# facebookresearch/DLRM-FlexFlow

Hardware: AMD Instinct MI355X
Metric: dlrm_training_samples_per_sec (higher is better)
Workload: dtype f32; 1 GPU; criteo-terabyte-shape: 26 tables (rows 39884406-39043-17289-7420-20263-3-7120-1543-63-38532951-2953546-403346-10-2208-11938-155-4-976-14-39979771-25641295-39664984-585935-12972-108-36), emb_dim 128, bag 1, bot 13-512-256-128, top 3456-1024-1024-512-256-1, cat interaction, SGD lr 0.01, MSE loss; global_batch=32768, per_gpu_batch=32768, parallelism=single GPU, hipGraph-replayed step, step_graph=True

## Files before the change

### dlrm_flexflow_amd/csrc/embedding.hip

```cpp
#include "emb_reduce.h"
#include "lr_state.h"

#include <type_traits>

namespace {

using namespace ffh_emb;

struct EmbArgs {
  ffh_emb_table t[FFH_MAX_TABLES];
  unsigned short* out16[FFH_MAX_TABLES];
  char* out3[FFH_MAX_TABLES];
  int   out3c[FFH_MAX_TABLES];
  int64_t batch;
  int     ntables;
  int     L;
  int     D;
  int     aggr;
  int64_t nt_rows;
};

template <int VEC, class WT> struct RowVec { typedef typename std::conditional<VEC == 4, float4, float>::type type; };
template <> struct RowVec<4, uint16_t> { typedef uint2 type; };
template <> struct RowVec<1, uint16_t> { typedef unsigned short type; };
template <int VEC, class WT>
__device__ __forceinline__ float row_elem(const typename RowVec<VEC, WT>::type& v, int k) {
  if constexpr (std::is_same<WT, float>::value) return reinterpret_cast<const float*>(&v)[k];
  else return ffh_bf16_to_f32(reinterpret_cast<const unsigned short*>(&v)[k]);
}

template <int VEC, int UNROLL, class WT = float>
__global__ __launch_bounds__(256) void emb_fwd_kernel(const EmbArgs a) {
  ffh_kernel_prio();
  using vec_t = typename RowVec<VEC, WT>::type;
  constexpr int NQ = VEC / 4;
  const ffh_emb_table tb = a.t[blockIdx.y];
  const WT* const wt = reinterpret_cast<const WT*>(tb.weight);
  unsigned short* const o16 = a.out16[blockIdx.y];
  char* const o3 = a.out3[blockIdx.y];
  const int o3c = a.out3c[blockIdx.y];
  const int D = a.D, L = a.L;
  const int nvec = D / VEC;
  const int lpr = nvec < 64 ? nvec : 64;
  const int rpw = 64 / lpr;
  const int lane = threadIdx.x & 63;
  const int wave = threadIdx.x >> 6;
  const int rsub = lane / lpr;
  const int c0 = lane - rsub * lpr;
  const bool active = rsub < rpw;
  const int64_t rows_per_block = (int64_t)(blockDim.x >> 6) * rpw * UNROLL;
  const float inv = 1.0f / (float)L;
  const bool avg = a.aggr == FFH_AGGR_MODE_AVG;

// ... 195 lines not shown
  if (vec == 4) hipLaunchKernelGGL((emb_fwd_kernel<4, U, WT>), grid, dim3(256), 0, as_stream(s), a);
  else hipLaunchKernelGGL((emb_fwd_kernel<1, U, WT>), grid, dim3(256), 0, as_stream(s), a);
  FFH_LAUNCH_CHECK(c, "emb_fwd_kernel");
  return FFH_OK;
}

extern "C" {

int ffh_embedding_fwd_multi(ffh_ctx* c, const ffh_emb_table* tables, int nt, int L, int D, int64_t batch, int aggr, ffh_stream s) {
  return emb_fwd_launch<float>(c, tables, nt, L, D, batch, aggr, s);
}

int ffh_embedding_fwd(ffh_ctx* c, const int64_t* idx, float* out, const float* weight, int L, int D, int64_t batch,
                      int64_t num_entries, int64_t out_ld, int aggr, ffh_stream s) {
  ffh_emb_table t{idx, const_cast<float*>(weight), out, num_entries, out_ld};
  return ffh_embedding_fwd_multi(c, &t, 1, L, D, batch, aggr, s);
}

int ffh_embedding_bwd_dense(ffh_ctx* c, const int64_t* idx, const float* g, float* wg, int L, int D, int64_t batch,
                            int64_t num_entries, int64_t gld, int aggr, ffh_stream s) {
  ffh_emb_table t{idx, wg, const_cast<float*>(g), num_entries, gld};
  int rc = validate_tables(c, &t, 1, L, D, batch, aggr, "embedding_bwd_dense");
  if (rc) return rc;
  if (batch == 0) return FFH_OK;
  hipLaunchKernelGGL(emb_bwd_dense_kernel, dim3(ffh_grid(batch * D, 256, 4096)), dim3(256), 0, as_stream(s),
                     idx, g, wg, L, D, batch, gld, aggr == FFH_AGGR_MODE_AVG ? 1 : 0);
  FFH_LAUNCH_CHECK(c, "emb_bwd_dense_kernel");
  return FFH_OK;
}

int ffh_embedding_localize_rows(ffh_ctx* c, const int64_t* idx, int64_t* local, int64_t n, int64_t row_begin, int64_t rows_local, ffh_stream s) {
  FFH_REQUIRE(c, n >= 0 && row_begin >= 0 && rows_local >= 0 && ((idx && local) || n == 0), "embedding_localize_rows: bad args");
  if (n == 0) return FFH_OK;
  hipLaunchKernelGGL(emb_localize_kernel, dim3(ffh_grid(n, 256)), dim3(256), 0, as_stream(s), idx, local, n, row_begin, rows_local);
  FFH_LAUNCH_CHECK(c, "embedding_localize_rows");
  return FFH_OK;
}

size_t ffh_embedding_bwd_workspace_bytes(int nt, int L, int D, int64_t batch) {
  if (nt <= 0 || L <= 0 || D <= 0 || batch <= 0) return 0;
  return bwd_layout(nt, L, D, batch).total;
}

struct Bf16Cfg { const ffh_bf16_rounding* r; Bf16Keys keys; };
typedef bool (*UpdateOfFn)(const UpdateLaunch&);
static constexpr UpdateOfFn kUpdateOf[2] = {emb_update_launch_f32, emb_update_launch_bf16};
static void set_bf16_keys(Bf16Keys& keys, Bf16AdamKeys& adam, const Bf16Cfg& b16, const ffh_emb_state* states, int nt, int kind) {
  if (kind != FFH_SPARSE_OPT_ADAM) { keys = b16.keys; return; }
  Bf16AdamKeys k;
  memset(&k, 0, sizeof k);
  for (int i = 0; i < nt; i++) { k.s1[i] = states[i].s1; k.table[i] = b16.keys.table[i]; k.col0[i] = b16.keys.col0[i]; }
  adam = k;
}
static int emb_bwd_phases(ffh_ctx* c, const ffh_emb_table* tables, int nt, int L, int D, int64_t batch,
                          int aggr, float lr, ffh_stream s, const bool do_sort, const bool do_apply,
                          const ffh_sparse_opt* opt = nullptr, const ffh_emb_state* states = nullptr, const Bf16Cfg* b16 = nullptr,
                          const ffh_lr_state* lr_block = nullptr) {
  int rc = validate_tables(c, tables, nt, L, D, batch, aggr, "embedding_bwd_sgd_fused");
  if (rc) return rc;
  OptP op{};
  op.lr = lr;
  if (b16 && do_apply) {
    const ffh_bf16_rounding* r = b16->r;
    if (!r) return ffh_fail(c, FFH_ERR_BAD_ARG, "embedding_bwd_bf16: null ffh_bf16_rounding");
    if (r->mode != FFH_BF16_ROUND_STOCHASTIC && r->mode != FFH_BF16_ROUND_NEAREST) return ffh_fail(c, FFH_ERR_BAD_ARG, "embedding_bwd_bf16: unknown rounding mode");
    if (r->mode == FFH_BF16_ROUND_STOCHASTIC && !r->counter) return ffh_fail(c, FFH_ERR_BAD_ARG, "embedding_bwd_bf16: stochastic rounding needs the update counter");
    op.sr_mode = r->mode; op.sr_seed = r->seed; op.sr_counter = r->counter;
  }
  op.nt_rows = (int64_t)FFH_LAB_INT("FFH_EMB_APPLY_NT_MB", 64) * (int64_t)(1 << 20) / ((int64_t)D * (b16 ? 2 : 4));
  int kind = FFH_SPARSE_OPT_SGD;
  RowRule rule = RowRule::Sgd;
  if (opt && do_apply) {
    kind = opt->kind;
    if (!row_rule_of(kind, &rule)) return ffh_fail(c, FFH_ERR_BAD_ARG, "embedding_bwd_opt: unknown ffh_sparse_opt.kind");
    if (b16 && (kind == FFH_SPARSE_OPT_SGD_MOMENTUM || kind == FFH_SPARSE_OPT_ADAM) && nt > FFH_BF16_MAX_STATEFUL_TABLES)
      return ffh_fail(c, FFH_ERR_BAD_ARG, "embedding_bwd_opt_multi_bf16: momentum / Adam take at most FFH_BF16_MAX_STATEFUL_TABLES (32) tables per call");
    op.lr = opt->lr; op.wd = opt->weight_decay; op.mom = opt->momentum; op.nesterov = opt->nesterov ? 1 : 0;
    op.b1 = opt->beta1; op.b2 = opt->beta2; op.eps = opt->epsilon; op.omb1 = 1.0f - opt->beta1; op.omb2 = 1.0f - opt->beta2;
    if (kind == FFH_SPARSE_OPT_SGD && (op.wd != 0.0f || op.mom != 0.0f)) return ffh_fail(c, FFH_ERR_BAD_ARG, "embedding_bwd_opt: FFH_SPARSE_OPT_SGD takes no weight decay / momentum (use FFH_SPARSE_OPT_SGD_MOMENTUM)");
    if (lr_block) { op.lr = 0.0f; opt_set_lr_src(op, ffh_lr_rate_ptr(lr_block, kind == FFH_SPARSE_OPT_ADAM)); }
    const bool need0 = kind == FFH_SPARSE_OPT_ADAM || kind == FFH_SPARSE_OPT_ADAGRAD || kind == FFH_SPARSE_OPT_ROWWISE_ADAGRAD || (kind == FFH_SPARSE_OPT_SGD_MOMENTUM && op.mom > 0.0f);
    for (int i = 0; i < nt && batch > 0; i++) {
      if (need0 && (!states || !states[i].s0)) return ffh_fail(c, FFH_ERR_BAD_ARG, "embedding_bwd_opt: optimizer state (s0) missing");
      if (kind == FFH_SPARSE_OPT_ADAM && !states[i].s1) return ffh_fail(c, FFH_ERR_BAD_ARG, "embedding_bwd_opt: optimizer state (s1) missing");
    }
  }
  if (nt == 0 || batch == 0) return FFH_OK;
  const int64_t N = batch * L;
  if (N >= (1LL << 31)) return ffh_fail(c, FFH_ERR_UNSUPPORTED, "embedding_bwd_sgd_fused: batch*in_dim >= 2^31");
  int64_t maxR = 1;
  for (int i = 0; i < nt; i++) maxR = tables[i].num_entries > maxR ? tables[i].num_entries : maxR;
  if (maxR > (1LL << 32)) return ffh_fail(c, FFH_ERR_UNSUPPORTED, "embedding_bwd_sgd_fused: num_entries > 2^32");
  bool v4 = can_vec4(tables, nt, D);
  for (int i = 0; i < nt && v4 && kind != FFH_SPARSE_OPT_SGD && kind != FFH_SPARSE_OPT_ROWWISE_ADAGRAD; i++)
    v4 = (!states[i].s0 || aligned16(states[i].s0)) && (kind == FFH_SPARSE_OPT_ADAGRAD || !states[i].s1 || aligned16(states[i].s1));
  const int nvec = v4 ? D / 4 : D;
  if ((nvec + 63) / 64 > kMaxChunks * 64) return ffh_fail(c, FFH_ERR_UNSUPPORTED, "embedding_bwd_sgd_fused: out_dim too large");
  if (kind == FFH_SPARSE_OPT_ROWWISE_ADAGRAD && (nvec + 63) / 64 > kMaxChunks)
    return ffh_fail(c, FFH_ERR_UNSUPPORTED, "embedding_bwd_opt: FFH_SPARSE_OPT_ROWWISE_ADAGRAD takes out_dim <= 1024 (16-byte form) / 256 (include/ff_hip_rowwise.h)");
  const BwdLayout lay = bwd_layout(nt, L, D, batch);
  if (!c->ws || c->ws_bytes < lay.total) return ffh_fail(c, FFH_ERR_WORKSPACE, "embedding_bwd_sgd_fused: workspace too small (ffh_embedding_bwd_workspace_bytes)");
  char* ws = (char*)c->ws;
  if (!aligned16(ws)) return ffh_fail(c, FFH_ERR_WORKSPACE, "embedding_bwd_sgd_fused: workspace must be 16-byte aligned");
  const int64_t sig[4] = {nt, L, D, batch};
  if (do_sort && do_apply) {
    if (c->emb_sorted_ws == c->ws) c->emb_sorted_ws = nullptr;
// ... 22 lines not shown
      while (tb < 32 && ((tables[i].num_entries - 1) >> tb) != 0) tb++;
      sm.npass[i] = (uint8_t)((tb + rb_s - 1) / rb_s);
    }
    sm.kp = (uint2*)(ws + lay.kp_a);
    sm.partial0 = (float*)(ws + lay.partial); sm.meta0 = (uint2*)(ws + lay.meta);
    sm.partial1 = (float*)(ws + lay.partial1); sm.meta1 = (uint2*)(ws + lay.meta1);
    sm.N = N; sm.nch0 = lay.nchunks; sm.nch1 = lay.nchunks1; sm.rb = rb_s; sm.L = L; sm.D = D;
    sm.avg = aggr == FFH_AGGR_MODE_AVG ? 1 : 0; sm.op = op;
    for (int i = 0; i < nt && kind != FFH_SPARSE_OPT_SGD; i++) { sm.s0[i] = states[i].s0; sm.s1[i] = states[i].s1; }
    if (b16) set_bf16_keys(sm.b16, sm.b16a, *b16, states, nt, kind);
    int tile = (int)((N + kSmallRedParts - 1) / kSmallRedParts);
    tile = (tile + FFH_EMB_CHUNK - 1) / FFH_EMB_CHUNK * FFH_EMB_CHUNK;
    sm.tile = tile < FFH_EMB_CHUNK ? FFH_EMB_CHUNK : tile;
    if (!kUpdateOf[b16 ? 1 : 0](UpdateLaunch{rule, v4, lr_block != nullptr, false, &sm, nullptr, dim3(nt), as_stream(s)}))
      return ffh_fail(c, FFH_ERR_UNSUPPORTED, "embedding_bwd: no small-batch kernel for this rule / weight type");
    FFH_LAUNCH_CHECK(c, "emb_sgd_small_kernel");
    return FFH_OK;
  }
  int bits = 1;
  while (bits < 32 && ((maxR - 1) >> bits) != 0) bits++;
  static const int msd_env = FFH_LAB_INT("FFH_EMB_MSD", 1);
  static const int msd_max_tables = FFH_LAB_INT("FFH_EMB_MSD_MAX_TABLES", FFH_MAX_TABLES);
  int mb = 4;
  while (mb < kMaxRadixBits && (N >> (mb + 1)) >= 32) mb++;
  const bool msd = msd_env != 0 && bits > kMaxRadixBits && N <= 65536 && (N >> mb) <= 128 && (msd_env == 2 || nt <= msd_max_tables) &&
                   (size_t)lay.nblk * kMaxRadix >= (size_t)lay.nchunks1;
  const int passes = msd ? 1 : (bits + kMaxRadixBits - 1) / kMaxRadixBits;
  const int rb = msd ? mb : (bits + passes - 1) / passes;
  if (msd) snprintf(c->emb_route, sizeof c->emb_route, "buckets:bits=%d", rb); else snprintf(c->emb_route, sizeof c->emb_route, "lsd:passes=%d", passes);

  SortArgs sa;
  memset(&sa, 0, sizeof sa);
  RedArgs ra;
  memset(&ra, 0, sizeof ra);
  for (int i = 0; i < nt; i++) {
    sa.idx[i] = tables[i].idx;
    int tb = 1;
    while (tb < 32 && ((tables[i].num_entries - 1) >> tb) != 0) tb++;
    const int np = msd ? 1 : (tb + rb - 1) / rb;
    sa.npass[i] = (uint8_t)np;
    ra.parity[i] = (uint8_t)(np & 1);
    sa.shift_t[i] = ra.shift_t[i] = (uint8_t)(msd && tb > rb ? tb - rb : 0);
  }
  sa.msd = msd ? 1 : 0;
  sa.bstart = (uint32_t*)(ws + lay.bstart);
  ra.bstart = sa.bstart; ra.nextkey = (uint32_t*)(ws + lay.hist); ra.radix = 1 << rb;
  sa.hist = (uint32_t*)(ws + lay.hist);
  sa.N = N; sa.nblk = lay.nblk; sa.bits = rb;
  sa.clear[0] = (uint32_t*)(ws + lay.meta1); sa.nclear[0] = 4 * lay.nchunks1;
  sa.clear[1] = (uint32_t*)(ws + lay.arrive); sa.nclear[1] = lay.nchunks1 + 1;
  uint2* kbuf[2] = {(uint2*)(ws + lay.kp_a), (uint2*)(ws + lay.kp_b)};
  dim3 sgrid((unsigned)lay.nblk, (unsigned)nt);
  const int E = sort_per_thread(nt, N);
  for (int p = 0; p < passes && do_sort; p++) {
    sa.shift = p * rb;
    sa.pass = p;
    sa.src = kbuf[p & 1];
    sa.dst = kbuf[(p + 1) & 1];
#define FFH_SORT_PASS(FIRSTV, EV)                                                                              \
    hipLaunchKernelGGL((radix_hist_kernel<FIRSTV, EV>), sgrid, dim3(kSortThreads), 0, as_stream(s), sa);      \
    hipLaunchKernelGGL((radix_scatter_kernel<FIRSTV, EV>), sgrid, dim3(kSortThreads), 0, as_stream(s), sa);
    if (p == 0) {
      switch (E) { case 1: FFH_SORT_PASS(true, 1) break; case 2: FFH_SORT_PASS(true, 2) break; case 4: FFH_SORT_PASS(true, 4) break; default: FFH_SORT_PASS(true, 8) break; }
    } else {
      switch (E) { case 1: FFH_SORT_PASS(false, 1) break; case 2: FFH_SORT_PASS(false, 2) break; case 4: FFH_SORT_PASS(false, 4) break; default: FFH_SORT_PASS(false, 8) break; }
    }
#undef FFH_SORT_PASS
  }
  FFH_LAUNCH_CHECK(c, "radix sort");
  if (!do_apply) return FFH_OK;

  for (int i = 0; i < nt; i++) ra.t[i] = tables[i];
  ra.kp[0] = kbuf[0]; ra.kp[1] = kbuf[1];
  ra.tile = reduce_tile(nt, N);
  {
    static const int msd_tile = FFH_LAB_INT("FFH_EMB_MSD_TILE", 0);
    if (msd && msd_tile >= 128 && msd_tile <= kRedTile && (msd_tile & (msd_tile - 1)) == 0) ra.tile = msd_tile;
  }
  ra.partial = (float*)(ws + lay.partial);
  ra.meta = (uint2*)(ws + lay.meta);
  ra.N = N; ra.nchunks = lay.nchunks; ra.L = L; ra.D = D;
  ra.avg = aggr == FFH_AGGR_MODE_AVG ? 1 : 0;
  ra.op = op;
  for (int i = 0; i < nt && kind != FFH_SPARSE_OPT_SGD; i++) { ra.s0[i] = states[i].s0; ra.s1[i] = states[i].s1; }
  if (b16) set_bf16_keys(ra.b16, ra.b16a, *b16, states, nt, kind);
  ra.partial1 = (float*)(ws + lay.partial1);
  ra.meta1 = (uint2*)(ws + lay.meta1); ra.nchunks1 = lay.nchunks1;
  ra.arrive = (uint32_t*)(ws + lay.arrive);
  dim3 rgrid((unsigned)((N + ra.tile - 1) / ra.tile), (unsigned)nt);
  if (!kUpdateOf[b16 ? 1 : 0](UpdateLaunch{rule, v4, lr_block != nullptr, msd, nullptr, &ra, rgrid, as_stream(s)}))
    return ffh_fail(c, FFH_ERR_UNSUPPORTED, "embedding_bwd: no reduce kernel for this rule / weight type");
  FFH_LAUNCH_CHECK(c, "emb_sgd_reduce/fold");
  return FFH_OK;
}

int ffh_embedding_bwd_sgd_fused_multi(ffh_ctx* c, const ffh_emb_table* tables, int nt, int L, int D, int64_t batch,
                                      int aggr, float lr, ffh_stream s) {
  return emb_bwd_phases(c, tables, nt, L, D, batch, aggr, lr, s, true, true);
}

int ffh_embedding_bwd_sort_multi(ffh_ctx* c, const ffh_emb_table* tables, int nt, int L, int D, int64_t batch, ffh_stream s) {
  return emb_bwd_phases(c, tables, nt, L, D, batch, FFH_AGGR_MODE_SUM, 0.0f, s, true, false);
}

int ffh_embedding_bwd_sgd_apply_multi(ffh_ctx* c, const ffh_emb_table* tables, int nt, int L, int D, int64_t batch,
                                      int aggr, float lr, ffh_stream s) {
  return emb_bwd_phases(c, tables, nt, L, D, batch, aggr, lr, s, false, true);
}

int ffh_embedding_bwd_opt_fused_multi(ffh_ctx* c, const ffh_emb_table* tables, const ffh_emb_state* states, int nt, int L, int D, int64_t batch,
                                      int aggr, const ffh_sparse_opt* opt, ffh_stream s) {
  if (!opt) return ffh_fail(c, FFH_ERR_BAD_ARG, "embedding_bwd_opt_fused_multi: null ffh_sparse_opt");
  return emb_bwd_phases(c, tables, nt, L, D, batch, aggr, opt->lr, s, true, true, opt, states);
}

int ffh_embedding_bwd_opt_apply_multi(ffh_ctx* c, const ffh_emb_table* tables, const ffh_emb_state* states, int nt, int L, int D, int64_t batch,
                                      int aggr, const ffh_sparse_opt* opt, ffh_stream s) {
  if (!opt) return ffh_fail(c, FFH_ERR_BAD_ARG, "embedding_bwd_opt_apply_multi: null ffh_sparse_opt");
  return emb_bwd_phases(c, tables, nt, L, D, batch, aggr, opt->lr, s, false, true, opt, states);
}

int ffh_embedding_bwd_opt_fused_multi_lr(ffh_ctx* c, const ffh_emb_table* tables, const ffh_emb_state* states, int nt, int L, int D, int64_t batch,
                                         int aggr, const ffh_sparse_opt* opt, const ffh_lr_state* block, ffh_stream s) {
  if (!opt || !block) return ffh_fail(c, FFH_ERR_BAD_ARG, "embedding_bwd_opt_fused_multi_lr: null ffh_sparse_opt or ffh_lr_state");
  return emb_bwd_phases(c, tables, nt, L, D, batch, aggr, 0.0f, s, true, true, opt, states, nullptr, block);
}

int ffh_embedding_bwd_opt_apply_multi_lr(ffh_ctx* c, const ffh_emb_table* tables, const ffh_emb_state* states, int nt, int L, int D, int64_t batch,
                                         int aggr, const ffh_sparse_opt* opt, const ffh_lr_state* block, ffh_stream s) {
  if (!opt || !block) return ffh_fail(c, FFH_ERR_BAD_ARG, "embedding_bwd_opt_apply_multi_lr: null ffh_sparse_opt or ffh_lr_state");
  return emb_bwd_phases(c, tables, nt, L, D, batch, aggr, 0.0f, s, false, true, opt, states, nullptr, block);
}

int ffh_embedding_bwd_sgd_fused(ffh_ctx* c, const int64_t* idx, const float* g, float* weight, int L, int D, int64_t batch,
                                int64_t num_entries, int64_t gld, int aggr, float lr, ffh_stream s) {
  ffh_emb_table t{idx, weight, const_cast<float*>(g), num_entries, gld};
  return ffh_embedding_bwd_sgd_fused_multi(c, &t, 1, L, D, batch, aggr, lr, s);
}

}

__global__ __launch_bounds__(256) void init_uniform_bf16_kernel(uint16_t* __restrict__ p, int64_t n, uint64_t seed, float lo, float hi) {
  const int64_t stride = (int64_t)gridDim.x * blockDim.x;
  for (int64_t i = (int64_t)blockIdx.x * blockDim.x + threadIdx.x; i < n; i += stride)
    p[i] = ffh_bf16_rne(ffh_uniform(ffh_hash(seed, (uint64_t)i), lo, hi));
}

__global__ void bf16_counter_advance_kernel(uint64_t* counter) { *counter = *counter + 1; }

static int bf16_tables(ffh_ctx* c, const ffh_emb_table_bf16* in, int nt, ffh_emb_table* out, Bf16Keys* keys) {
  if (nt < 0 || nt > FFH_MAX_TABLES) return ffh_fail(c, FFH_ERR_BAD_ARG, "embedding_bf16: ntables out of range");
  if (nt > 0 && !in) return ffh_fail(c, FFH_ERR_BAD_ARG, "embedding_bf16: null tables");
  for (int i = 0; i < nt; i++) {
    if (in[i].table < 0 || in[i].col0 < 0) return ffh_fail(c, FFH_ERR_BAD_ARG, "embedding_bf16: negative table index or col0");
    out[i] = ffh_emb_table{in[i].idx, reinterpret_cast<float*>(in[i].weight), in[i].io, in[i].num_entries, in[i].ld};
    if (keys) { keys->table[i] = in[i].table; keys->col0[i] = in[i].col0; }
  }
  return FFH_OK;
}

static int emb_bwd_bf16(ffh_ctx* c, const ffh_emb_table_bf16* tables, int nt, int L, int D, int64_t batch, int aggr, float lr,
                        const ffh_bf16_rounding* r, ffh_stream s, bool do_sort, bool do_apply,
                        const ffh_sparse_opt* opt = nullptr, const ffh_emb_state* states = nullptr, const ffh_lr_state* lr_block = nullptr) {
  ffh_emb_table t[FFH_MAX_TABLES];
  Bf16Cfg cfg;
  memset(&cfg, 0, sizeof cfg);
  cfg.r = r;
  const int rc = bf16_tables(c, tables, nt, t, &cfg.keys);
  if (rc) return rc;
  return emb_bwd_phases(c, t, nt, L, D, batch, aggr, lr, s, do_sort, do_apply, opt, states, &cfg, lr_block);
}

extern "C" {

int ffh_bf16_abi_version(void) { return FFH_BF16_ABI_VERSION; }

int ffh_embedding_fwd_multi_bf16(ffh_ctx* c, const ffh_emb_table_bf16* tables, int nt, int L, int D, int64_t batch, int aggr, ffh_stream s) {
  ffh_emb_table t[FFH_MAX_TABLES];
  const int rc = bf16_tables(c, tables, nt, t, nullptr);
  if (rc) return rc;
  return emb_fwd_launch<uint16_t>(c, t, nt, L, D, batch, aggr, s);
}

int ffh_embedding_bwd_sgd_fused_multi_bf16(ffh_ctx* c, const ffh_emb_table_bf16* tables, int nt, int L, int D, int64_t batch,
                                           int aggr, float lr, const ffh_bf16_rounding* r, ffh_stream s) {
  return emb_bwd_bf16(c, tables, nt, L, D, batch, aggr, lr, r, s, true, true);
}

int ffh_embedding_bwd_sort_multi_bf16(ffh_ctx* c, const ffh_emb_table_bf16* tables, int nt, int L, int D, int64_t batch, ffh_stream s) {
  return emb_bwd_bf16(c, tables, nt, L, D, batch, FFH_AGGR_MODE_SUM, 0.0f, nullptr, s, true, false);
}

int ffh_embedding_bwd_sgd_apply_multi_bf16(ffh_ctx* c, const ffh_emb_table_bf16* tables, int nt, int L, int D, int64_t batch,
                                           int aggr, float lr, const ffh_bf16_rounding* r, ffh_stream s) {
// ... 49 lines not shown
```

### dlrm_flexflow_amd/csrc/fold.hip

```cpp
#include "linear_gemm.h"

#include "../../include/ff_hip_fold.h"

using namespace ffh_gemm;

namespace {

typedef float f32x4 __attribute__((ext_vector_type(4)));

struct FoldGemmGroup { const float* a; int64_t lda; int64_t wcol0; float* c; int64_t ldc; int rows; int tile0; };
struct FoldGemmArgs {
  FoldGemmGroup grp[FFH_FOLD_MAX_GROUPS];
  ffh_fold_seg  seg[FFH_FOLD_MAX_SEGS];
  const float*  w; int64_t ldw;
  const float*  bias;
  const float*  addend; int64_t ldadd;
  int ngroups, nseg, N, act, ntiles;
};
static_assert(sizeof(FoldGemmArgs) <= 4096, "kernel arguments");

template <bool EPI>
__global__ __launch_bounds__(256) void fold_gemm_kernel(const FoldGemmArgs g) {
  ffh_kernel_prio();
  const int lane = threadIdx.x & 63;
  const int wave = __builtin_amdgcn_readfirstlane((int)(threadIdx.x >> 6));
  const int c = lane & 15, q = lane >> 4;
  const int wt = (int)blockIdx.x * 4 + wave;
  if (wt >= g.ntiles) return;
  int gi = 0;
  while (gi + 1 < g.ngroups && g.grp[gi + 1].tile0 <= wt) gi++;
  const FoldGemmGroup G = g.grp[gi];
  const int ct = g.N / 64, local = wt - G.tile0;
  const int r0 = (local / ct) * 32, n0 = (local % ct) * 64;
  const float* ap[2];
  const float* wp[4];
#pragma unroll
  for (int mt = 0; mt < 2; mt++) {
    int r = r0 + 16 * mt + c;
    if (r > G.rows - 1) r = G.rows - 1;
    ap[mt] = G.a + (int64_t)r * G.lda + 4 * q;
  }
#pragma unroll
  for (int nt = 0; nt < 4; nt++) wp[nt] = g.w + (int64_t)(n0 + 16 * nt + c) * g.ldw + G.wcol0 + 4 * q;
  f32x4 acc[4][2];
#pragma unroll
  for (int nt = 0; nt < 4; nt++)
#pragma unroll
    for (int mt = 0; mt < 2; mt++) acc[nt][mt] = f32x4{0.f, 0.f, 0.f, 0.f};
  for (int si = 0; si < g.nseg; si++) {
    const int k0 = g.seg[si].k0, k1 = k0 + g.seg[si].len;
    for (int k = k0; k < k1; k += 16) {
      f32x4 a[2], b[4];
// ... 246 lines not shown
  a.S = S; a.ldS = ldS; a.batch = batch; a.ntables = ntables; a.L = in_dim; a.out = out;
  hipLaunchKernelGGL(fold_gather_add_kernel, dim3(ffh_grid(batch * (out / 4), 256, 4096)), dim3(256), 0, as_stream(s), a);
  FFH_LAUNCH_CHECK(c, "fold_gather_add_kernel");
  return FFH_OK;
}

int ffh_fold_linear_fwd_plan(ffh_ctx* c, const float* x, int64_t ldx, const float* y, int64_t ldy, const float* w, const float* bias, int in, int out,
                             int64_t batch, const ffh_fold_seg* keep, int nkeep, const float* addend, int64_t ldadd) {
  const int rc = fold_fwd_check(c, x, ldx, y, ldy, w, in, out, batch, keep, nkeep, addend, ldadd);
  if (rc != FFH_OK) return rc;
  if (!fold_fwd_served(c, x, ldx, y, ldy, w, in, out, keep, nkeep, addend, ldadd)) return ffh_fail(c, FFH_ERR_UNSUPPORTED, "fold_linear_fwd: shape / alignment / math mode not served");
  const GemmArgs g = fold_fwd_gemm(x, ldx, const_cast<float*>(y), ldy, w, bias, in, out, batch, FFH_AC_MODE_NONE);
  unsigned long long mask[2]; int nk = 0;
  if (batch > 0 && fold_keep_mask(in, keep, nkeep, mask, &nk) && launch_gemm_sk_fold(c, g, mask, nk, addend, ldadd, true, nullptr, "") == 1) return 2;
  return (batch > 0 && gemm_sk_serves(c, g, SK_FORM_FWD)) ? 0 : 1;
}

int ffh_fold_linear_fwd(ffh_ctx* c, const float* x, int64_t ldx, float* y, int64_t ldy, const float* w, const float* bias, int in, int out, int64_t batch,
                        int act, const ffh_fold_seg* keep, int nkeep, const float* addend, int64_t ldadd, ffh_stream s) {
  if (nkeep == 0 && !addend) return ffh_linear_fwd(c, x, ldx, y, ldy, w, bias, in, out, batch, act, s);
  const int rc = fold_fwd_check(c, x, ldx, y, ldy, w, in, out, batch, keep, nkeep, addend, ldadd);
  if (rc != FFH_OK) return rc;
  if (act != FFH_AC_MODE_NONE && act != FFH_AC_MODE_RELU && act != FFH_AC_MODE_SIGMOID && act != FFH_AC_MODE_GELU)
    return ffh_fail(c, FFH_ERR_UNSUPPORTED, "fold_linear_fwd: activation not supported (NONE, RELU, SIGMOID, GELU)");
  if (!fold_fwd_served(c, x, ldx, y, ldy, w, in, out, keep, nkeep, addend, ldadd)) return ffh_fail(c, FFH_ERR_UNSUPPORTED, "fold_linear_fwd: shape / alignment / math mode not served");
  ffh_route_clear(c);
  if (batch == 0) return FFH_OK;
  const GemmArgs g = fold_fwd_gemm(x, ldx, y, ldy, w, bias, in, out, batch, act);
  unsigned long long mask[2]; int nk = 0;
  if (fold_keep_mask(in, keep, nkeep, mask, &nk) && (!bias || al16(bias))) {
    const int r = launch_gemm_sk_fold(c, g, mask, nk, addend, ldadd, false, s, "fold_linear_fwd gemm");
    if (r != 0) return r < 0 ? r : FFH_OK;
  }
  FoldGemmArgs a{};
  a.grp[0] = FoldGemmGroup{x, ldx, 0, y, ldy, (int)batch, 0};
  if (nkeep == 0) { a.seg[0] = ffh_fold_seg{0, in}; a.nseg = 1; }
  else { for (int i = 0; i < nkeep; i++) a.seg[i] = keep[i]; a.nseg = nkeep; }
  const int64_t tiles = ((batch + 31) / 32) * (out / 64);
  FFH_REQUIRE(c, tiles < (1LL << 30), "fold_linear_fwd: too many tiles");
  a.w = w; a.ldw = in; a.bias = bias; a.addend = addend; a.ldadd = ldadd; a.ngroups = 1; a.N = out; a.act = act; a.ntiles = (int)tiles;
  hipLaunchKernelGGL(fold_gemm_kernel<true>, dim3((unsigned)((tiles + 3) / 4)), dim3(256), 0, as_stream(s), a);
  FFH_LAUNCH_CHECK(c, "fold_gemm_kernel (forward)");
  ffh_route_add(c, "fold_linear_fwd gemm|mfma_32x64x16");
  return FFH_OK;
}

int ffh_fold_segment_sum(ffh_ctx* c, const ffh_emb_table* tables, int ntables, int in_dim, int width, int64_t batch, ffh_stream s) {
  FFH_REQUIRE(c, tables && ntables >= 1 && in_dim >= 1 && width > 0 && batch >= 0, "fold_segment_sum: bad arguments");
  if (ntables > FFH_MAX_TABLES || batch * in_dim >= (1LL << 31)) return ffh_fail(c, FFH_ERR_UNSUPPORTED, "fold_segment_sum: at most 64 tables, batch * in_dim < 2^31");
  for (int t = 0; t < ntables; t++)
    FFH_REQUIRE(c, tables[t].weight && tables[t].num_entries >= 1 && (batch == 0 || (tables[t].idx && tables[t].io && tables[t].ld >= width)), "fold_segment_sum: bad table");
  if (batch > 0 && (!c->ws || c->ws_bytes < ffh_embedding_bwd_workspace_bytes(ntables, in_dim, width, batch) || ((uintptr_t)c->ws & 15)))
    return ffh_fail(c, FFH_ERR_WORKSPACE, "fold_segment_sum: workspace too small (ffh_embedding_bwd_workspace_bytes) or not 16-byte aligned");
  for (int t = 0; t < ntables;) {
    char* p0 = (char*)tables[t].weight;
    size_t bytes = 0;
    for (; t < ntables && (char*)tables[t].weight == p0 + bytes; t++) bytes += (size_t)tables[t].num_entries * (size_t)width * 4;
    const int rc = ffh_zero(c, p0, bytes, s);
    if (rc != FFH_OK) return rc;
  }
  if (batch == 0) return FFH_OK;
  return ffh_embedding_bwd_sgd_fused_multi(c, tables, ntables, in_dim, width, batch, FFH_AGGR_MODE_SUM, -1.0f, s);
}

int ffh_fold_dw_product(ffh_ctx* c, const ffh_fold_group* groups, int ngroups, float* dw, int64_t lddw, int d, int out, ffh_stream s) {
  FFH_REQUIRE(c, groups && dw && ngroups >= 1 && d > 0 && out > 0 && lddw >= d, "fold_dw_product: bad arguments");
  if (ngroups > FFH_FOLD_MAX_GROUPS || d % 64 || out % FFH_FOLD_NTILE) return ffh_fail(c, FFH_ERR_UNSUPPORTED, "fold_dw_product: d and out_dim multiples of 64, at most 64 tables");
  FoldDwArgs a{};
  int64_t tiles = 0;
  for (int i = 0; i < ngroups; i++) {
    const ffh_fold_group& gr = groups[i];
    FFH_REQUIRE(c, gr.e && gr.p && gr.rows >= 1 && gr.rows < (1LL << 31) && gr.lde >= d && gr.col0 >= 0 && gr.col0 + d <= lddw, "fold_dw_product: bad group");
    if (!al16(gr.e) || !al16(gr.p) || gr.lde % 4) return ffh_fail(c, FFH_ERR_UNSUPPORTED, "fold_dw_product: group not aligned");
    a.grp[i] = FoldDwGroup{gr.p, gr.e, gr.lde, gr.col0, (int)gr.rows, (int)tiles};
    tiles += ((gr.rows + FFH_FOLD_DW_CHUNK - 1) / FFH_FOLD_DW_CHUNK) * (out / 64) * (d / 64);
    FFH_REQUIRE(c, tiles < (1LL << 30), "fold_dw_product: too many rows");
  }
  a.dw = dw; a.lddw = lddw; a.ngroups = ngroups; a.out = out; a.d = d; a.ntiles = (int)tiles;
  hipLaunchKernelGGL(fold_dw_product_kernel, dim3((unsigned)((tiles + 3) / 4)), dim3(256), 0, as_stream(s), a);
  FFH_LAUNCH_CHECK(c, "fold_dw_product_kernel");
  return FFH_OK;
}

int ffh_fold_linear_bwd_dw_plan(ffh_ctx* c, const float* x, int64_t ldx, const float* dy, int64_t lddy, const float* dw, const float* db, int in, int out,
                                int64_t batch, const int32_t* kept, int nkept) {
  const int rc = fold_dw_check(c, x, ldx, dy, lddy, dw, in, out, batch, kept, nkept);
  if (rc != FFH_OK) return rc;
  if (batch == 0 || c->math_mode != FFH_MATH_DEFAULT) return 0;
  const GemmArgs g = fold_dw_gemm(x, ldx, dy, lddy, const_cast<float*>(dw), const_cast<float*>(db), in, out, batch);
  if (!gemm_sk_serves(c, g, SK_FORM_DW)) return 0;
  return launch_gemm_sk_kept(c, g, kept, nkept, true, nullptr, "") == 1 ? 1 : 0;
}

int ffh_fold_linear_bwd_dw(ffh_ctx* c, const float* x, int64_t ldx, const float* dy, int64_t lddy, float* dw, float* db, int in, int out, int64_t batch,
                           const int32_t* kept, int nkept, ffh_stream s) {
  const int rc = fold_dw_check(c, x, ldx, dy, lddy, dw, in, out, batch, kept, nkept);
  if (rc != FFH_OK) return rc;
  ffh_route_clear(c);
  if (batch == 0 || c->math_mode != FFH_MATH_DEFAULT) return ffh_fail(c, FFH_ERR_UNSUPPORTED, "fold_linear_bwd_dw: empty batch / math mode not served");
  const GemmArgs g = fold_dw_gemm(x, ldx, dy, lddy, dw, db, in, out, batch);
  if (!gemm_sk_serves(c, g, SK_FORM_DW)) return ffh_fail(c, FFH_ERR_UNSUPPORTED, "fold_linear_bwd_dw: the layer's weight gradient does not run the stream-K form");
  const int r = launch_gemm_sk_kept(c, g, kept, nkept, false, s, "fold_linear_bwd_dw gemm");
  if (r < 0) return r;
  if (r == 0) return ffh_fail(c, FFH_ERR_UNSUPPORTED, "fold_linear_bwd_dw: too few kept tiles for the stream-K form, deterministic mode, or a bias gradient without tile 0");
  return FFH_OK;
}
// ... 3 lines not shown
```

Baseline: 4.792 million samples/s.

## Add wide fold segment-sum path with fused zeroing and sorted block reduction

Adds a dedicated fold_sum_wide path for ffh_fold_segment_sum when the width is a multiple of 256. It sorts the keys fully, then runs a block kernel that sums runs of sorted gradient rows, writes each row directly and zeros the untouched rows in the same pass. A join kernel then combines runs that cross block boundaries. This replaces the separate full-table memset plus the generic SGD-fused reduce, cutting a large zeroing pass and extra launches, at the cost of new, complex boundary-handling code.

Measured after the change: 4.842 million samples/s, median of 6. +1.0%, better.

```diff
diff --git a/dlrm_flexflow_amd/csrc/embedding.hip b/dlrm_flexflow_amd/csrc/embedding.hip
--- a/dlrm_flexflow_amd/csrc/embedding.hip
+++ b/dlrm_flexflow_amd/csrc/embedding.hip
@@ -1,4 +1,5 @@
 #include "emb_reduce.h"
+#include "fold_sum.h"
 #include "lr_state.h"
 
 #include <type_traits>
@@ -300,6 +301,24 @@
   for (int i = 0; i < nt; i++) { k.s1[i] = states[i].s1; k.table[i] = b16.keys.table[i]; k.col0[i] = b16.keys.col0[i]; }
   adam = k;
 }
+static void launch_sort_passes(SortArgs& sa, uint2* const kbuf[2], int passes, int rb, int E, dim3 sgrid, ffh_stream s) {
+  for (int p = 0; p < passes; p++) {
+    sa.shift = p * rb;
+    sa.pass = p;
+    sa.src = kbuf[p & 1];
+    sa.dst = kbuf[(p + 1) & 1];
+#define FFH_SORT_PASS(FIRSTV, EV)                                                                              \
+    hipLaunchKernelGGL((radix_hist_kernel<FIRSTV, EV>), sgrid, dim3(kSortThreads), 0, as_stream(s), sa);      \
+    hipLaunchKernelGGL((radix_scatter_kernel<FIRSTV, EV>), sgrid, dim3(kSortThreads), 0, as_stream(s), sa);
+    if (p == 0) {
+      switch (E) { case 1: FFH_SORT_PASS(true, 1) break; case 2: FFH_SORT_PASS(true, 2) break; case 4: FFH_SORT_PASS(true, 4) break; default: FFH_SORT_PASS(true, 8) break; }
+    } else {
+      switch (E) { case 1: FFH_SORT_PASS(false, 1) break; case 2: FFH_SORT_PASS(false, 2) break; case 4: FFH_SORT_PASS(false, 4) break; default: FFH_SORT_PASS(false, 8) break; }
+    }
+#undef FFH_SORT_PASS
+  }
+}
+
 static int emb_bwd_phases(ffh_ctx* c, const ffh_emb_table* tables, int nt, int L, int D, int64_t batch,
                           int aggr, float lr, ffh_stream s, const bool do_sort, const bool do_apply,
                           const ffh_sparse_opt* opt = nullptr, const ffh_emb_state* states = nullptr, const Bf16Cfg* b16 = nullptr,
@@ -428,21 +447,7 @@
   uint2* kbuf[2] = {(uint2*)(ws + lay.kp_a), (uint2*)(ws + lay.kp_b)};
   dim3 sgrid((unsigned)lay.nblk, (unsigned)nt);
   const int E = sort_per_thread(nt, N);
-  for (int p = 0; p < passes && do_sort; p++) {
-    sa.shift = p * rb;
-    sa.pass = p;
-    sa.src = kbuf[p & 1];
-    sa.dst = kbuf[(p + 1) & 1];
-#define FFH_SORT_PASS(FIRSTV, EV)                                                                              \
-    hipLaunchKernelGGL((radix_hist_kernel<FIRSTV, EV>), sgrid, dim3(kSortThreads), 0, as_stream(s), sa);      \
-    hipLaunchKernelGGL((radix_scatter_kernel<FIRSTV, EV>), sgrid, dim3(kSortThreads), 0, as_stream(s), sa);
-    if (p == 0) {
-      switch (E) { case 1: FFH_SORT_PASS(true, 1) break; case 2: FFH_SORT_PASS(true, 2) break; case 4: FFH_SORT_PASS(true, 4) break; default: FFH_SORT_PASS(true, 8) break; }
-    } else {
-      switch (E) { case 1: FFH_SORT_PASS(false, 1) break; case 2: FFH_SORT_PASS(false, 2) break; case 4: FFH_SORT_PASS(false, 4) break; default: FFH_SORT_PASS(false, 8) break; }
-    }
-#undef FFH_SORT_PASS
-  }
+  if (do_sort) launch_sort_passes(sa, kbuf, passes, rb, E, sgrid, s);
   FFH_LAUNCH_CHECK(c, "radix sort");
   if (!do_apply) return FFH_OK;
 
@@ -516,6 +521,41 @@
 
 }
 
+int ffh_emb::emb_sort_full(ffh_ctx* c, const ffh_emb_table* tables, int nt, int L, int D, int64_t batch, ffh_stream s, FullSort* out) {
+  const int64_t N = batch * L;
+  const BwdLayout lay = bwd_layout(nt, L, D, batch);
+  char* ws = (char*)c->ws;
+  if (c->emb_sorted_ws == c->ws) c->emb_sorted_ws = nullptr;
+  int64_t maxR = 1;
+  for (int i = 0; i < nt; i++) maxR = tables[i].num_entries > maxR ? tables[i].num_entries : maxR;
+  if (maxR > (1LL << 32)) return ffh_fail(c, FFH_ERR_UNSUPPORTED, "fold_segment_sum: num_entries > 2^32");
+  int bits = 1;
+  while (bits < 32 && ((maxR - 1) >> bits) != 0) bits++;
+  const int passes = (bits + kMaxRadixBits - 1) / kMaxRadixBits;
+  const int rb = (bits + passes - 1) / passes;
+  SortArgs sa;
+  memset(&sa, 0, sizeof sa);
+  uint2* kbuf[2] = {(uint2*)(ws + lay.kp_a), (uint2*)(ws + lay.kp_b)};
+  for (int i = 0; i < nt; i++) {
+    sa.idx[i] = tables[i].idx;
+    int tb = 1;
+    while (tb < 32 && ((tables[i].num_entries - 1) >> tb) != 0) tb++;
+    const int np = (tb + rb - 1) / rb;
+    sa.npass[i] = (uint8_t)np;
+    out->kp[i] = kbuf[np & 1] + (int64_t)i * N;
+  }
+  sa.bstart = (uint32_t*)(ws + lay.bstart);
+  sa.hist = (uint32_t*)(ws + lay.hist);
+  sa.N = N; sa.nblk = lay.nblk; sa.bits = rb;
+  sa.clear[0] = (uint32_t*)(ws + lay.meta1); sa.clear[1] = (uint32_t*)(ws + lay.arrive);
+  launch_sort_passes(sa, kbuf, passes, rb, sort_per_thread(nt, N), dim3((unsigned)lay.nblk, (unsigned)nt), s);
+  FFH_LAUNCH_CHECK(c, "radix sort");
+  out->partial0 = (float*)(ws + lay.partial);
+  out->partial1 = (float*)(ws + lay.partial1);
+  out->passes = passes;
+  return FFH_OK;
+}
+
 __global__ __launch_bounds__(256) void init_uniform_bf16_kernel(uint16_t* __restrict__ p, int64_t n, uint64_t seed, float lo, float hi) {
   const int64_t stride = (int64_t)gridDim.x * blockDim.x;
   for (int64_t i = (int64_t)blockIdx.x * blockDim.x + threadIdx.x; i < n; i += stride)
diff --git a/dlrm_flexflow_amd/csrc/fold.hip b/dlrm_flexflow_amd/csrc/fold.hip
--- a/dlrm_flexflow_amd/csrc/fold.hip
+++ b/dlrm_flexflow_amd/csrc/fold.hip
@@ -1,3 +1,4 @@
+#include "fold_sum.h"
 #include "linear_gemm.h"
 
 #include "../../include/ff_hip_fold.h"
@@ -350,6 +351,10 @@
     FFH_REQUIRE(c, tables[t].weight && tables[t].num_entries >= 1 && (batch == 0 || (tables[t].idx && tables[t].io && tables[t].ld >= width)), "fold_segment_sum: bad table");
   if (batch > 0 && (!c->ws || c->ws_bytes < ffh_embedding_bwd_workspace_bytes(ntables, in_dim, width, batch) || ((uintptr_t)c->ws & 15)))
     return ffh_fail(c, FFH_ERR_WORKSPACE, "fold_segment_sum: workspace too small (ffh_embedding_bwd_workspace_bytes) or not 16-byte aligned");
+  if (batch > 0) {
+    const int wide = ffh_emb::fold_sum_wide(c, tables, ntables, in_dim, width, batch, s);
+    if (wide != 0) return wide < 0 ? wide : FFH_OK;
+  }
   for (int t = 0; t < ntables;) {
     char* p0 = (char*)tables[t].weight;
     size_t bytes = 0;
diff --git a/dlrm_flexflow_amd/csrc/fold_sum.h b/dlrm_flexflow_amd/csrc/fold_sum.h
--- /dev/null
+++ b/dlrm_flexflow_amd/csrc/fold_sum.h
@@ -0,0 +1,17 @@
+#pragma once
+#include "ffh_common.h"
+
+namespace ffh_emb {
+
+struct FullSort {
+  const uint2* kp[FFH_MAX_TABLES];
+  float*       partial0;
+  float*       partial1;
+  int          passes;
+};
+
+__attribute__((visibility("hidden"))) int emb_sort_full(ffh_ctx* c, const ffh_emb_table* tables, int nt, int L, int D, int64_t batch, ffh_stream s, FullSort* out);
+
+__attribute__((visibility("hidden"))) int fold_sum_wide(ffh_ctx* c, const ffh_emb_table* tables, int nt, int L, int width, int64_t batch, ffh_stream s);
+
+}
diff --git a/dlrm_flexflow_amd/csrc/fold_sum.hip b/dlrm_flexflow_amd/csrc/fold_sum.hip
--- /dev/null
+++ b/dlrm_flexflow_amd/csrc/fold_sum.hip
@@ -0,0 +1,228 @@
+#include "fold_sum.h"
+
+#include "../../include/ff_hip_fold.h"
+
+#include <utility>
+
+using namespace ffh_emb;
+
+namespace {
+
+typedef float f32x4 __attribute__((ext_vector_type(4)));
+
+constexpr int kFsSlice = 256;
+constexpr int kFsBlock = FFH_EMB_CHUNK1;
+constexpr int kFsChunk = FFH_EMB_CHUNK;
+constexpr int kFsWaves = 4;
+static_assert(kFsChunk == 32, "a 32-block's entries are held by lanes 0..31 of a wave, its two neighbours by lanes 32 and 33");
+
+struct FoldSumTable { const uint2* kp; const float* dy; int64_t ld; float* g; int64_t rows; };
+struct FoldSumArgs {
+  FoldSumTable t[FFH_MAX_TABLES];
+  float*  partial0;
+  float*  partial;
+  int64_t N, nchunks;
+  int L, width, nblk1, nslices;
+};
+static_assert(sizeof(FoldSumArgs) <= 4096, "kernel arguments");
+
+__device__ __forceinline__ uint32_t uni(uint32_t v) { return __builtin_amdgcn_readfirstlane(v); }
+
+template <int... I, class F>
+__device__ __forceinline__ void fs_static_for_impl(std::integer_sequence<int, I...>, F&& f) { (f(std::integral_constant<int, I>{}), ...); }
+template <int N_, class F>
+__device__ __forceinline__ void fs_static_for(F&& f) { fs_static_for_impl(std::make_integer_sequence<int, N_>{}, static_cast<F&&>(f)); }
+
+template <int Q>
+__device__ __forceinline__ void fs_issue(f32x4 (&v)[16], const float* dyc, int64_t ld, uint32_t brow, int n) {
+#pragma unroll
+  for (int u = 0; u < 8; u++)
+    if (8 * Q + u < n) v[8 * (Q & 1) + u] = *reinterpret_cast<const f32x4*>(dyc + (int64_t)__builtin_amdgcn_readlane(brow, 8 * Q + u) * ld);
+}
+
+__global__ __launch_bounds__(256) void fold_sum_block_kernel(const FoldSumArgs a) {
+  __shared__ uint32_t s_key[kFsBlock];
+  ffh_kernel_prio();
+  const int lane = threadIdx.x & 63;
+  const int wave = (int)uni(threadIdx.x >> 6);
+  const int t = blockIdx.y;
+  const int slice = (int)(blockIdx.x % (unsigned)a.nslices), blk = (int)(blockIdx.x / (unsigned)a.nslices);
+  const FoldSumTable T = a.t[t];
+  const int64_t N = a.N, base = (int64_t)blk * kFsBlock;
+  const int cnt = (int)(N - base < kFsBlock ? N - base : kFsBlock);
+  const int nb32 = (cnt + kFsChunk - 1) / kFsChunk;
+  const int col = slice * kFsSlice + 4 * lane;
+  const float* const dyc = T.dy + col;
+  float* const gc = T.g + col;
+  float* const pc = a.partial + ((int64_t)t * a.nblk1 + blk) * 2 * a.width + col;
+  float* const p0 = a.partial0 + ((int64_t)t * a.nchunks + base / kFsChunk) * 2 * a.width + col;
+  const int L = a.L;
+
+  const bool cont_prev = blk > 0 && T.kp[base - 1].x == T.kp[base].x;
+  const bool cont_next = base + cnt < N && T.kp[base + cnt].x == T.kp[base + cnt - 1].x;
+
+  auto fetch = [&](int B, uint2& kp, bool& ok) {
+    const int64_t e = base + (int64_t)B * kFsChunk + (lane < 32 ? lane : lane == 32 ? -1 : kFsChunk);
+    ok = lane < 34 && B < nb32 && e >= 0 && e < N;
+    kp = ok ? T.kp[e] : make_uint2(0u, 0u);
+  };
+  auto count_of = [&](int B) { return B >= nb32 ? 0 : cnt - B * kFsChunk < kFsChunk ? cnt - B * kFsChunk : kFsChunk; };
+  auto dy_row = [&](uint32_t pos) { return L == 1 ? pos : pos / (uint32_t)L; };
+
+  uint2 kp_cur, kp_nxt;
+  bool ok_cur, ok_nxt;
+  fetch(wave, kp_cur, ok_cur);
+  fetch(wave + kFsWaves, kp_nxt, ok_nxt);
+  f32x4 v[16];
+  fs_issue<0>(v, dyc, T.ld, dy_row(kp_cur.y), count_of(wave));
+  fs_issue<1>(v, dyc, T.ld, dy_row(kp_cur.y), count_of(wave));
+
+  for (int B = wave; B < nb32; B += kFsWaves) {
+    const unsigned long long okm = __ballot(ok_cur);
+    const uint32_t key = kp_cur.x, brow = dy_row(kp_cur.y);
+    const int n = count_of(B);
+    if (lane < n) s_key[B * kFsChunk + lane] = key;
+    const uint32_t k_first = __builtin_amdgcn_readlane(key, 0), k_last = __builtin_amdgcn_readlane(key, n - 1);
+    const bool prev_same = ((okm >> 32) & 1) && (uint32_t)__builtin_amdgcn_readlane(key, 32) == k_first;
+    const bool next_same = ((okm >> 33) & 1) && (uint32_t)__builtin_amdgcn_readlane(key, 33) == k_last;
+    const bool in_prev = B > 0, in_next = B < nb32 - 1;
+
+    auto close = [&](uint32_t row, const f32x4 acc, bool at_start, bool at_end) {
+      const bool from_left = at_start && prev_same, to_right = at_end && next_same;
+      float* dst;
+      if (from_left && in_prev) dst = p0 + (int64_t)(2 * B) * a.width;
+      else if (to_right && in_next) dst = p0 + (int64_t)(2 * B + 1) * a.width;
+      else dst = from_left ? pc : to_right ? pc + a.width : gc + (int64_t)row * a.width;
+      *reinterpret_cast<f32x4*>(dst) = acc;
+    };
+    auto zero_rows = [&](int64_t lo, int64_t hi) {
+      for (int64_t r = lo; r < hi; r++) *reinterpret_cast<f32x4*>(gc + r * a.width) = f32x4{0.f, 0.f, 0.f, 0.f};
+    };
+    if (!prev_same) zero_rows(((okm >> 32) & 1) ? (int64_t)(uint32_t)__builtin_amdgcn_readlane(key, 32) + 1 : 0, k_first);
+    if (base + (int64_t)B * kFsChunk + n == N) zero_rows((int64_t)k_last + 1, T.rows);
+    f32x4 acc = v[0];
+    uint32_t row = k_first;
+    bool at_start = true;
+    fs_static_for<kFsChunk>([&](auto jc) {
+      constexpr int j = jc + 1;
+      if constexpr (j == 16) { fs_issue<2>(v, dyc, T.ld, brow, n); fs_issue<3>(v, dyc, T.ld, brow, n); }
+      if constexpr (j < kFsChunk) {
+        if (j < n) {
+          const uint32_t kj = __builtin_amdgcn_readlane(key, j);
+          if (kj != row) {
+            close(row, acc, at_start, false);
+            zero_rows((int64_t)row + 1, kj);
+            acc = v[j & 15]; row = kj; at_start = false;
+          } else {
+            acc += v[j & 15];
+          }
+        }
+      }
+      if constexpr (j == 32) { fs_issue<0>(v, dyc, T.ld, dy_row(kp_nxt.y), count_of(B + kFsWaves)); fs_issue<1>(v, dyc, T.ld, dy_row(kp_nxt.y), count_of(B + kFsWaves)); }
+    });
+    close(row, acc, at_start, true);
+    kp_cur = kp_nxt; ok_cur = ok_nxt;
+    fetch(B + 2 * kFsWaves, kp_nxt, ok_nxt);
+  }
+  __syncthreads();
+
+  auto last_of = [&](int B) { const int e = B * kFsChunk + kFsChunk - 1; return uni(s_key[e < cnt ? e : cnt - 1]); };
+  for (int B = wave; B < nb32 - 1; B += kFsWaves) {
+    const uint32_t first = uni(s_key[B * kFsChunk]), row = last_of(B);
+    if (row != uni(s_key[(B + 1) * kFsChunk])) continue;
+    if (B > 0 && first == row && uni(s_key[B * kFsChunk - 1]) == row) continue;
+    int B2 = B + 1;
+    while (B2 < nb32 - 1 && last_of(B2) == row && uni(s_key[(B2 + 1) * kFsChunk]) == row) B2++;
+    f32x4 acc = *reinterpret_cast<const f32x4*>(p0 + (int64_t)(2 * B + 1) * a.width);
+    for (int b0 = B + 1; b0 <= B2; b0 += 8) {
+      f32x4 p[8];
+#pragma unroll
+      for (int u = 0; u < 8; u++)
+        if (b0 + u <= B2) p[u] = *reinterpret_cast<const f32x4*>(p0 + (int64_t)(2 * (b0 + u)) * a.width);
+#pragma unroll
+      for (int u = 0; u < 8; u++)
+        if (b0 + u <= B2) acc += p[u];
+    }
+    const bool from_left = cont_prev && uni(s_key[0]) == row, to_right = cont_next && uni(s_key[cnt - 1]) == row;
+    float* dst = from_left ? pc : to_right ? pc + a.width : gc + (int64_t)row * a.width;
+    *reinterpret_cast<f32x4*>(dst) = acc;
+  }
+}
+
+__global__ __launch_bounds__(64) void fold_sum_join_kernel(const FoldSumArgs a) {
+  ffh_kernel_prio();
+  const int lane = threadIdx.x;
+  const int t = blockIdx.y;
+  const FoldSumTable T = a.t[t];
+  const int64_t N = a.N;
+  const int col = (int)blockIdx.x * kFsSlice + 4 * lane;
+  const float* const part = a.partial + (int64_t)t * a.nblk1 * 2 * a.width + col;
+  float* const gc = T.g + col;
+  f32x4 acc = f32x4{0.f, 0.f, 0.f, 0.f};
+  for (int k0 = 0; k0 < a.nblk1; k0 += 4) {
+    uint32_t key = 0;
+    bool ok = false;
+    {
+      const int k = k0 + (lane >> 2), j = lane & 3;
+      if (lane < 16 && k < a.nblk1) {
+        const int64_t b0 = (int64_t)k * kFsBlock, b1 = b0 + kFsBlock < N ? b0 + kFsBlock : N;
+        const int64_t e = j == 0 ? b0 - 1 : j == 1 ? b0 : j == 2 ? b1 - 1 : b1;
+        ok = e >= 0 && e < N;
+        if (ok) key = T.kp[e].x;
+      }
+    }
+    const unsigned long long okm = __ballot(ok);
+    f32x4 vl[4], vr[4];
+    uint32_t first[4];
+    bool open_l[4], open_r[4], through[4];
+#pragma unroll
+    for (int i = 0; i < 4; i++) {
+      const int k = k0 + i;
+      open_l[i] = open_r[i] = through[i] = false;
+      first[i] = 0;
+      if (k < a.nblk1) {
+        first[i] = __builtin_amdgcn_readlane(key, 4 * i + 1);
+        const uint32_t last = __builtin_amdgcn_readlane(key, 4 * i + 2);
+        open_l[i] = ((okm >> (4 * i)) & 1) && (uint32_t)__builtin_amdgcn_readlane(key, 4 * i) == first[i];
+        open_r[i] = ((okm >> (4 * i + 3)) & 1) && (uint32_t)__builtin_amdgcn_readlane(key, 4 * i + 3) == last;
+        through[i] = open_l[i] && open_r[i] && first[i] == last;
+        if (open_l[i]) vl[i] = *reinterpret_cast<const f32x4*>(part + (int64_t)(2 * k) * a.width);
+        if (open_r[i] && !through[i]) vr[i] = *reinterpret_cast<const f32x4*>(part + (int64_t)(2 * k + 1) * a.width);
+      }
+    }
+#pragma unroll
+    for (int i = 0; i < 4; i++) {
+      if (open_l[i]) {
+        acc += vl[i];
+        if (!through[i]) *reinterpret_cast<f32x4*>(gc + (int64_t)first[i] * a.width) = acc;
+      }
+      if (open_r[i] && !through[i]) acc = vr[i];
+    }
+  }
+}
+
+inline bool al16(const void* p) { return ((uintptr_t)p & 15) == 0; }
+
+}
+
+int ffh_emb::fold_sum_wide(ffh_ctx* c, const ffh_emb_table* tables, int nt, int L, int width, int64_t batch, ffh_stream s) {
+  if (width % kFsSlice) return 0;
+  for (int t = 0; t < nt; t++)
+    if (!al16(tables[t].weight) || !al16(tables[t].io) || tables[t].ld % 4) return 0;
+  FullSort srt;
+  const int rc = emb_sort_full(c, tables, nt, L, width, batch, s, &srt);
+  if (rc != FFH_OK) return rc;
+  FoldSumArgs a;
+  memset(&a, 0, sizeof a);
+  for (int t = 0; t < nt; t++) a.t[t] = FoldSumTable{srt.kp[t], tables[t].io, tables[t].ld, tables[t].weight, tables[t].num_entries};
+  a.partial0 = srt.partial0; a.partial = srt.partial1;
+  a.N = batch * L; a.L = L; a.width = width;
+  a.nblk1 = (int)((a.N + kFsBlock - 1) / kFsBlock);
+  a.nchunks = (a.N + kFsChunk - 1) / kFsChunk;
+  a.nslices = width / kFsSlice;
+  hipLaunchKernelGGL(fold_sum_block_kernel, dim3((unsigned)a.nblk1 * (unsigned)a.nslices, (unsigned)nt), dim3(64 * kFsWaves), 0, as_stream(s), a);
+  if (a.nblk1 > 1) hipLaunchKernelGGL(fold_sum_join_kernel, dim3((unsigned)a.nslices, (unsigned)nt), dim3(64), 0, as_stream(s), a);
+  FFH_LAUNCH_CHECK(c, "fold_sum_block_kernel / fold_sum_join_kernel");
+  snprintf(c->emb_route, sizeof c->emb_route, "fold_sum:wide|slice=%d|lsd:passes=%d", kFsSlice, srt.passes);
+  return 1;
+}
```
